# zc402/video-classification

Hardware: AMD Instinct MI355X
Metric: clips/sec SlowFast-R50 8x8, 32x224^2 bf16 training step (higher is better)
Workload: dtype bf16

## Files before the change

video-classification_amd/build.py:

```python
import os
import subprocess
from concurrent.futures import ThreadPoolExecutor

HERE = os.path.dirname(os.path.abspath(__file__))
ROOT = os.path.dirname(HERE)
CSRC = os.path.join(HERE, "csrc")
LIB = os.path.join(HERE, "libsfk.so")
SOURCES = ["conv_igemm.hip", "conv_igemm_p8.hip", "conv_halo.hip", "conv_pw.hip", "conv_wgrad.hip", "conv_wgrad_p8.hip", "conv_wgrad_band.hip", "stem_conv.hip", "bn.hip", "bn_tail.hip", "pool_head.hip",
           "optim_misc.hip", "eval_input.hip", "stem2d.hip", "roi_resize.hip", "sgd.hip", "color_jitter.hip", "u8_pool_gather.hip", "pad_resize.hip", "optim_sched.hip", "optim_groups.hip"]


def _newer(a, b):
    return (not os.path.exists(b)) or os.path.getmtime(a) > os.path.getmtime(b)


def build(force: bool = False, verbose: bool = False) -> str:
    hipcc = os.environ.get("HIPCC", "/opt/rocm/bin/hipcc")
    if not os.path.exists(hipcc):
        hipcc = "hipcc"
    objdir = os.path.join(HERE, "build")
    os.makedirs(objdir, exist_ok=True)
    deps = [os.path.join(CSRC, "sfk_common.h"), os.path.join(CSRC, "conv_igemm_epi.h"), os.path.join(CSRC, "conv_wgrad_common.h"), os.path.join(CSRC, "conv_wgrad_band_acc.inc"), os.path.join(ROOT, "include", "sfk.h"),
            os.path.join(ROOT, "include", "sfk_stem2d.h"), os.path.join(ROOT, "include", "sfk_u8stem.h"),
            os.path.join(ROOT, "include", "sfk_v2.h"), os.path.join(ROOT, "include", "sfk_aug.h"),
            os.path.join(ROOT, "include", "sfk_pool.h"), os.path.join(ROOT, "include", "sfk_resize.h"),
            os.path.join(ROOT, "include", "sfk_resident.h"), os.path.join(ROOT, "include", "sfk_roi_pool.h"),
            os.path.join(ROOT, "include", "sfk_roi_ragged.h"), os.path.join(ROOT, "include", "sfk_u8stem_pool.h"),
            os.path.join(ROOT, "include", "sfk_optim.h"), os.path.join(ROOT, "include", "sfk_groups.h"),
            os.path.join(CSRC, "optim_elem.h")]
    flags = ["--offload-arch=gfx950", "-O3", "-fPIC", "-std=c++17", "-I" + os.path.join(ROOT, "include"), "-I" + CSRC]
    flags += os.environ.get("SFK_EXTRA_FLAGS", "").split()

    def compile_one(src):
        s = os.path.join(CSRC, src)
        o = os.path.join(objdir, src.replace(".hip", ".o"))
        if force or _newer(s, o) or any(_newer(d, o) for d in deps):
            cmd = [hipcc] + flags + ["-c", s, "-o", o]
            if verbose:
                print(" ".join(cmd))
            subprocess.run(cmd, check=True)
            return o, True
        return o, False

    with ThreadPoolExecutor(max_workers=min(4, len(SOURCES))) as ex:
        res = list(ex.map(compile_one, SOURCES))
    objs = [o for o, _ in res]
    if force or any(ch for _, ch in res) or not os.path.exists(LIB):
        subprocess.run([hipcc, "--offload-arch=gfx950", "-shared", "-fPIC", "-o", LIB] + objs, check=True)
    return LIB


if __name__ == "__main__":
    print(build(force="--force" in os.sys.argv, verbose=True))
```

video-classification_amd/csrc/bn.hip:

```cpp
#include "sfk_common.h"


namespace {
inline int nt_hint(const sfk_fmap* f, int64_t mb, int bits) {
  const int64_t bytes = sfk_fmap_pixels(f) * f->c * (f->dtype == SFK_BF16 ? 2 : 4);
  return (mb >= 0 && bytes >= (mb << 20)) ? bits : 0;
}

struct FM {
  void* p;
  int ld, off;
};
inline FM fm_of(const sfk_fmap* f) { return FM{f ? f->ptr : nullptr, f ? f->ld : 0, f ? f->c_off : 0}; }

struct ChanMap {
  int cg, row, rows_b;
  bool active;
  __device__ __forceinline__ ChanMap(int cgs) {
    const int cgs_b = cgs < 256 ? cgs : 256;
    rows_b = 256 / cgs_b;
    const int tx = threadIdx.x % cgs_b, ty = threadIdx.x / cgs_b;
    cg = blockIdx.y * 256 + tx;
    row = ty;
    active = ty < rows_b && cg < cgs;
  }
};

#ifndef SFK_BN_U_ROWS
#define SFK_BN_U_ROWS 4
#endif
constexpr int SFK_BN_U = SFK_BN_U_ROWS;
inline unsigned span_blocks(int cgs, int64_t pixels) {
  const int cgs_b = cgs < 256 ? cgs : 256, rows_b = 256 / cgs_b;
  const int64_t want = (pixels + (int64_t)rows_b * SFK_BN_U - 1) / ((int64_t)rows_b * SFK_BN_U);
  return (unsigned)(want < 65535 ? (want > 0 ? want : 1) : 65535);
}
inline dim3 chan_grid(int cgs, int64_t pixels, int max_parts, int* nparts) {
  const int cgs_b = cgs < 256 ? cgs : 256;
  const int rows_b = 256 / cgs_b;
  int64_t parts = (pixels + (int64_t)rows_b * 16 - 1) / ((int64_t)rows_b * 16);
  const int cchunks = (cgs + 255) / 256;
  const int cap_all = sfk_tune().bn_parts;
  int64_t cap = cap_all / cchunks;
  if (cap < 1) cap = 1;
  if (parts > cap) parts = cap;
  if (max_parts > 0 && parts > max_parts) parts = max_parts;
  if (parts < 1) parts = 1;
  *nparts = (int)parts;
  return dim3((unsigned)parts, (unsigned)cchunks);
}

template <int VEC>
__device__ __forceinline__ void load_coef(float (&dst)[VEC], const float* src, int cg) {
#pragma unroll
  for (int i = 0; i < VEC; ++i) dst[i] = src[cg * VEC + i];
}

template <int VEC>
__device__ __forceinline__ void block_reduce_store(const ChanMap& cm, int cgs, const float (&a)[VEC],
                                                   const float (&b)[VEC], float* partials, int c) {
  __shared__ float red[256 * 2 * VEC];
  float* mine = red + threadIdx.x * 2 * VEC;
#pragma unroll
  for (int i = 0; i < VEC; ++i) {
    mine[2 * i] = cm.active ? a[i] : 0.f;
    mine[2 * i + 1] = cm.active ? b[i] : 0.f;
  }
  __syncthreads();
  const int cgs_b = cgs < 256 ? cgs : 256;
  const int W = cgs_b * 2 * VEC, rows = cm.rows_b, tid = threadIdx.x;
  float* out = partials + (int64_t)blockIdx.x * c * 2 + (int64_t)blockIdx.y * 256 * VEC * 2;
  const int ncol = (cgs - (int)blockIdx.y * 256 < cgs_b ? cgs - (int)blockIdx.y * 256 : cgs_b) * 2 * VEC;
  if (W >= 256) {
    for (int col = tid; col < W; col += 256) {
      float sacc = 0.f;
      for (int r = 0; r < rows; ++r) sacc += red[r * W + col];
      if (col < ncol) out[col] = sacc;
    }
    return;
  }
  const int G = 256 / W;
  const int g = tid / W, col = tid - g * W;
  float sacc = 0.f;
// ... 429 lines not shown
        c1[i] = coef[(cm.cg * VEC + i) * 3 + 1];
        c2[i] = coef[(cm.cg * VEC + i) * 3 + 2];
      }
    }
    const T* gp = static_cast<const T*>(dout.p) + dout.off + cm.cg * VEC;
    const uint8_t* ap = argmax + cm.cg * VEC;
    const T* yp = static_cast<const T*>(y.p) + y.off + cm.cg * VEC;
    T* op = APPLY ? static_cast<T*>(dyo.p) + dyo.off + cm.cg * VEC : nullptr;
    for (int64_t q = (int64_t)blockIdx.x * cm.rows_b + cm.row; q < quads; q += (int64_t)gridDim.x * cm.rows_b) {
      uint32_t q1, b, nt, a;
      g.dqw.divmod((uint32_t)q, q1, b);
      g.dqh.divmod(q1, nt, a);
      Vec16<T> gw[4], v[4];
      uint32_t alo[4], ahi[4];
      bool wok[4], pok[4];
#pragma unroll
      for (int wa = 0; wa < 2; ++wa)
#pragma unroll
        for (int wb = 0; wb < 2; ++wb) {
          const int ho = (int)a + wa, wo = (int)b + wb, k = 2 * wa + wb;
          wok[k] = ho < g.Ho && wo < g.Wo;
          const int hc = ho < g.Ho ? ho : g.Ho - 1, wc = wo < g.Wo ? wo : g.Wo - 1;
          const int64_t opix = ((int64_t)nt * g.Ho + hc) * g.Wo + wc;
          gw[k].load(gp + opix * dout.ld);
          const uint8_t* aq = ap + opix * c;
          if (VEC == 8) {
            const uint2 a2 = *reinterpret_cast<const uint2*>(aq);
            alo[k] = a2.x;
            ahi[k] = a2.y;
          } else {
            alo[k] = *reinterpret_cast<const uint32_t*>(aq);
            ahi[k] = 0;
          }
        }
      int64_t ipix[4];
#pragma unroll
      for (int ra = 0; ra < 2; ++ra)
#pragma unroll
        for (int rb = 0; rb < 2; ++rb) {
          const int hi = 2 * (int)a + ra, wi = 2 * (int)b + rb, k = 2 * ra + rb;
          pok[k] = hi < g.H && wi < g.W;
          const int hc = hi < g.H ? hi : g.H - 1, wc = wi < g.W ? wi : g.W - 1;
          ipix[k] = ((int64_t)nt * g.H + hc) * g.W + wc;
          v[k].load(yp + ipix[k] * y.ld);
        }
#pragma unroll
      for (int ra = 0; ra < 2; ++ra)
#pragma unroll
        for (int rb = 0; rb < 2; ++rb) {
          const int k = 2 * ra + rb;
          if (!pok[k]) continue;
          Vec16<T> da, o;
#pragma unroll
          for (int i = 0; i < VEC; ++i) {
            float acc = 0.f;
#pragma unroll
            for (int wa = 0; wa <= ra; ++wa)
#pragma unroll
              for (int wb = 0; wb <= rb; ++wb) {
                const int w4 = 2 * wa + wb;
                const uint32_t code = (uint32_t)((1 + ra - 2 * wa) * 3 + (1 + rb - 2 * wb));
                const uint32_t am = ((i < 4 ? alo[w4] : ahi[w4]) >> (8 * (i & 3))) & 0xFFu;
                if (wok[w4] && am == code) acc += gw[w4].get(i);
              }
            da.set(i, acc);
          }
#pragma unroll
          for (int i = 0; i < VEC; ++i) {
            const float yv = v[k].get(i);
            const float dz = (yv * sc[i] + sh[i] > 0.f) ? da.get(i) : 0.f;
            const float xh = (yv - mu[i]) * is[i];
            if (APPLY) {
              o.set(i, c0[i] * (dz - c1[i] - xh * c2[i]));
            } else {
              s1[i] += dz;
              s2[i] += dz * xh;
            }
          }
          if (APPLY) o.store(op + ipix[k] * dyo.ld);
        }
    }
  }
  if (!APPLY) block_reduce_store<VEC>(cm, cgs, s1, s2, partials, c);
}

bool same_shape(const sfk_fmap* a, const sfk_fmap* b) {
  return a->n == b->n && a->t == b->t && a->h == b->h && a->w == b->w && a->c == b->c && a->dtype == b->dtype;
}

}

extern "C" int sfk_bn_stats(const sfk_fmap* y, float* partials, int32_t max_parts, int32_t* nparts_out,
                            sfk_stream_t stream) {
  if (!sfk_fmap_ok(y) || !partials || !nparts_out || max_parts <= 0) return SFK_ERR_INVALID;
  if (!sfk_fmap_vec_ok(y)) return SFK_ERR_UNSUPPORTED;
  const int64_t px = sfk_fmap_pixels(y);
  int np;
  const dim3 grid = chan_grid(y->c / sfk_vec_of(y->dtype), px, max_parts, &np);
  hipStream_t s = static_cast<hipStream_t>(stream);
  if (y->dtype == SFK_BF16) hipLaunchKernelGGL(bn_stats_kernel<bf16_t>, grid, dim3(256), 0, s, fm_of(y), px, y->c, partials);
  else hipLaunchKernelGGL(bn_stats_kernel<float>, grid, dim3(256), 0, s, fm_of(y), px, y->c, partials);
  SFK_CHECK_LAUNCH();
  *nparts_out = np;
  return SFK_OK;
}

extern "C" int sfk_bn_finalize(const float* partials, int32_t nparts, int32_t c, int64_t count, const float* gamma,
                               const float* beta, float eps, float momentum, float* running_mean,
                               float* running_var, int64_t* num_batches_tracked, float* mean, float* invstd,
                               float* scale, float* shift, float* workspace, sfk_stream_t stream) {
  if (!partials || nparts <= 0 || c <= 0 || count <= 0 || !gamma || !beta || !mean || !invstd || !scale || !shift)
    return SFK_ERR_INVALID;
  if ((running_mean == nullptr) != (running_var == nullptr)) return SFK_ERR_INVALID;
  if (c & 1) return SFK_ERR_UNSUPPORTED;
  if ((((uintptr_t)partials) | ((uintptr_t)workspace)) & 15) return SFK_ERR_INVALID;
  hipStream_t s = static_cast<hipStream_t>(stream);
  partials = fold_partials(partials, nparts, c, workspace, &nparts, s);
  const FinK f{partials, nparts, c, (double)count, gamma, beta, eps, momentum, running_mean, running_var, num_batches_tracked,
               mean, invstd, scale, shift};
  hipLaunchKernelGGL(bn_finalize_kernel, dim3(c / 2), dim3(256), 0, s, f);
  SFK_CHECK_LAUNCH();
  return SFK_OK;
}

extern "C" int sfk_bn_eval_coeffs(const float* gamma, const float* beta, const float* running_mean,
                                  const float* running_var, float eps, int32_t c, float* scale, float* shift,
                                  sfk_stream_t stream) {
  if (!gamma || !beta || !running_mean || !running_var || !scale || !shift || c <= 0) return SFK_ERR_INVALID;
  hipLaunchKernelGGL(bn_eval_coeffs_kernel, dim3((c + 63) / 64), dim3(64), 0, static_cast<hipStream_t>(stream), gamma,
                     beta, running_mean, running_var, eps, c, scale, shift);
  SFK_CHECK_LAUNCH();
  return SFK_OK;
}

namespace {
template <typename T>
int launch_apply(const sfk_fmap* y, const float* scale, const float* shift, const sfk_fmap* res,
                 const float* rs, const float* rb, int relu, const sfk_fmap* out, uint8_t* bits, float* sums, int max_parts,
                 int* nparts_out, hipStream_t s) {
  const int64_t px = sfk_fmap_pixels(y);
  int np;
  dim3 grid = chan_grid(y->c / DT<T>::VEC, px, sums ? max_parts : 0, &np);
  const dim3 blk(256);
  const FM fy = fm_of(y), fr = fm_of(res), fo = fm_of(out);
  const int mode = !res ? 0 : (rs ? 2 : 1);
  const int nt = nt_hint(y, sfk_tune().nt_apply_mb, 3);
  if (sums) {
    if (mode != 0 || !relu) return SFK_ERR_UNSUPPORTED;
    if (nt) hipLaunchKernelGGL((bn_apply_kernel<T, 0, true, 3, true>), grid, blk, 0, s, fy, fr, fo, px, y->c, scale, shift, rs, rb, bits, sums);
    else hipLaunchKernelGGL((bn_apply_kernel<T, 0, true, 0, true>), grid, blk, 0, s, fy, fr, fo, px, y->c, scale, shift, rs, rb, bits, sums);
    SFK_CHECK_LAUNCH();
    *nparts_out = np;
    return SFK_OK;
  }
  grid.x = span_blocks(y->c / DT<T>::VEC, px);
#define SFK_APPLY(R, A)                                                                                                      \
  do {                                                                                                                     \
    if (nt) hipLaunchKernelGGL((bn_apply_kernel<T, R, A, 3>), grid, blk, 0, s, fy, fr, fo, px, y->c, scale, shift, rs, rb, bits); \
    else hipLaunchKernelGGL((bn_apply_kernel<T, R, A, 0>), grid, blk, 0, s, fy, fr, fo, px, y->c, scale, shift, rs, rb, bits);    \
  } while (0)
  if (relu) {
    if (mode == 0) SFK_APPLY(0, true); else if (mode == 1) SFK_APPLY(1, true); else SFK_APPLY(2, true);
  } else {
    if (mode == 0) SFK_APPLY(0, false); else if (mode == 1) SFK_APPLY(1, false); else SFK_APPLY(2, false);
  }
#undef SFK_APPLY
// ... 108 lines not shown
                                   float* workspace, sfk_stream_t stream) {
  if (!partials || nparts <= 0 || c <= 0 || count <= 0 || !gamma || !invstd || !coef) return SFK_ERR_INVALID;
  if (c & 1) return SFK_ERR_UNSUPPORTED;
  if ((((uintptr_t)partials) | ((uintptr_t)workspace)) & 15) return SFK_ERR_INVALID;
  hipStream_t s = static_cast<hipStream_t>(stream);
  partials = fold_partials(partials, nparts, c, workspace, &nparts, s);
  const BFinK f{partials, nparts, c, (double)count, gamma, invstd, dgamma, dbeta, coef};
  hipLaunchKernelGGL(bn_bwd_finalize_kernel, dim3(c / 2), dim3(256), 0, s, f);
  SFK_CHECK_LAUNCH();
  return SFK_OK;
}

extern "C" int sfk_bn_bwd_apply(const sfk_fmap* da, const sfk_fmap* y, const sfk_fmap* mask_src, const float* mean,
                                const float* invstd, const float* scale, const float* shift, int32_t relu,
                                const float* coef, const sfk_fmap* dy, sfk_stream_t stream) {
  const int st = check_bwd(da, y, mask_src, mean, invstd, scale, shift, relu);
  if (st != SFK_OK) return st;
  if (!coef || !sfk_fmap_ok(dy) || !same_shape(da, dy)) return SFK_ERR_INVALID;
  if (!sfk_fmap_vec_ok(dy)) return SFK_ERR_UNSUPPORTED;
  hipStream_t s = static_cast<hipStream_t>(stream);
  return y->dtype == SFK_BF16
             ? launch_bwd_apply<bf16_t>(da, y, mask_src, mean, invstd, scale, shift, relu, coef, dy, s)
             : launch_bwd_apply<float>(da, y, mask_src, mean, invstd, scale, shift, relu, coef, dy, s);
}

namespace {
int bn_pool_check(const sfk_fmap* d_out, const uint8_t* argmax, const sfk_fmap* y, const float* mean, const float* invstd,
                  const float* scale, const float* shift) {
  if (!sfk_fmap_ok(d_out) || !sfk_fmap_ok(y) || !argmax || !mean || !invstd || !scale || !shift) return SFK_ERR_INVALID;
  if (d_out->dtype != y->dtype || d_out->n != y->n || d_out->t != y->t || d_out->c != y->c) return SFK_ERR_INVALID;
  if (d_out->h != (y->h + 2 - 3) / 2 + 1 || d_out->w != (y->w + 2 - 3) / 2 + 1) return SFK_ERR_INVALID;
  if (!sfk_fmap_vec_ok(d_out) || !sfk_fmap_vec_ok(y)) return SFK_ERR_UNSUPPORTED;
  if (sfk_fmap_pixels(y) >= (1ll << 31)) return SFK_ERR_UNSUPPORTED;
  return SFK_OK;
}
inline PoolGeo pool_geo(const sfk_fmap* d_out, const sfk_fmap* y) {
  PoolGeo g;
  g.H = y->h; g.W = y->w; g.Ho = d_out->h; g.Wo = d_out->w;
  g.qh = (y->h + 1) / 2; g.qw = (y->w + 1) / 2;
  g.dqw.set(g.qw); g.dqh.set(g.qh);
  return g;
}
inline int64_t pool_quads(const sfk_fmap* y, const PoolGeo& g) { return (int64_t)y->n * y->t * g.qh * g.qw; }
}

extern "C" int sfk_bn_maxpool_bwd_reduce(const sfk_fmap* d_out, const uint8_t* argmax, const sfk_fmap* y, const float* mean,
                                         const float* invstd, const float* scale, const float* shift, float* partials,
                                         int32_t max_parts, int32_t* nparts_out, sfk_stream_t stream) {
  const int st = bn_pool_check(d_out, argmax, y, mean, invstd, scale, shift);
  if (st != SFK_OK) return st;
  if (!partials || !nparts_out || max_parts <= 0) return SFK_ERR_INVALID;
  const int64_t px = sfk_fmap_pixels(y);
  int np;
  const dim3 grid = chan_grid(y->c / sfk_vec_of(y->dtype), px, max_parts, &np);
  hipStream_t s = static_cast<hipStream_t>(stream);
  const PoolGeo g = pool_geo(d_out, y);
  const int64_t quads = pool_quads(y, g);
  if (y->dtype == SFK_BF16)
    hipLaunchKernelGGL((bn_pool_bwd_kernel<bf16_t, false>), grid, dim3(256), 0, s, fm_of(d_out), argmax, fm_of(y), FM{nullptr, 0, 0},
                       quads, y->c, g, mean, invstd, scale, shift, nullptr, partials);
  else
    hipLaunchKernelGGL((bn_pool_bwd_kernel<float, false>), grid, dim3(256), 0, s, fm_of(d_out), argmax, fm_of(y), FM{nullptr, 0, 0},
                       quads, y->c, g, mean, invstd, scale, shift, nullptr, partials);
  SFK_CHECK_LAUNCH();
  *nparts_out = np;
  return SFK_OK;
}

extern "C" int sfk_bn_maxpool_bwd_apply(const sfk_fmap* d_out, const uint8_t* argmax, const sfk_fmap* y, const float* mean,
                                        const float* invstd, const float* scale, const float* shift, const float* coef,
                                        const sfk_fmap* dy, sfk_stream_t stream) {
  const int st = bn_pool_check(d_out, argmax, y, mean, invstd, scale, shift);
  if (st != SFK_OK) return st;
  if (!coef || !sfk_fmap_ok(dy) || !same_shape(y, dy)) return SFK_ERR_INVALID;
  if (!sfk_fmap_vec_ok(dy)) return SFK_ERR_UNSUPPORTED;
  const int cgs = y->c / sfk_vec_of(y->dtype);
  const int cgs_b = cgs < 256 ? cgs : 256, rows_b = 256 / cgs_b;
  const PoolGeo g = pool_geo(d_out, y);
  const int64_t quads = pool_quads(y, g);
  int64_t want = (quads + rows_b - 1) / rows_b;
  if (want > 65535 * 16) want = 65535 * 16;
  const dim3 grid((unsigned)(want > 0 ? want : 1), (unsigned)((cgs + 255) / 256));
  hipStream_t s = static_cast<hipStream_t>(stream);
  if (y->dtype == SFK_BF16)
    hipLaunchKernelGGL((bn_pool_bwd_kernel<bf16_t, true>), grid, dim3(256), 0, s, fm_of(d_out), argmax, fm_of(y), fm_of(dy), quads,
                       y->c, g, mean, invstd, scale, shift, coef, nullptr);
  else
    hipLaunchKernelGGL((bn_pool_bwd_kernel<float, true>), grid, dim3(256), 0, s, fm_of(d_out), argmax, fm_of(y), fm_of(dy), quads,
                       y->c, g, mean, invstd, scale, shift, coef, nullptr);
  SFK_CHECK_LAUNCH();
  return SFK_OK;
}
```

video-classification_amd/csrc/pool_head.hip:

```cpp
#include "sfk_common.h"

namespace {

struct FM {
  void* p;
  int t, h, w, ld, off;
};
inline FM fm_of(const sfk_fmap* f) { return FM{f->ptr, f->t, f->h, f->w, f->ld, f->c_off}; }

template <typename T, int KC = 0, int SC = 0, int PC = 0, bool BN = false>
__global__ __launch_bounds__(256) void maxpool_fwd_kernel(FM x, FM y, uint8_t* argmax, int n, int c, int k_, int s_,
                                                          int p_, FastDiv dcg, FastDiv dwo, FastDiv dho,
                                                          const float* __restrict__ scale,
                                                          const float* __restrict__ shift) {
  const int k = KC ? KC : k_, s = KC ? SC : s_, p = KC ? PC : p_;
  constexpr int VEC = DT<T>::VEC;
  const int cgs = c / VEC;
  const int64_t total = (int64_t)n * y.t * y.h * y.w * cgs;
  for (int64_t idx = (int64_t)blockIdx.x * 256 + threadIdx.x; idx < total; idx += (int64_t)gridDim.x * 256) {
    uint32_t pix, cg, q1, wo, nt, ho;
    dcg.divmod((uint32_t)idx, pix, cg);
    dwo.divmod(pix, q1, wo);
    dho.divmod(q1, nt, ho);
    float best[VEC];
    int arg[VEC];
    float sc[VEC], sh[VEC];
#pragma unroll
    for (int i = 0; i < VEC; ++i) {
      best[i] = -INFINITY;
      arg[i] = 0;
      sc[i] = BN ? scale[cg * VEC + i] : 1.f;
      sh[i] = BN ? shift[cg * VEC + i] : 0.f;
    }
    bool first = true;
    if (KC) {
      Vec16<T> v[(KC ? KC : 1) * (KC ? KC : 1)];
#pragma unroll
      for (int kh = 0; kh < (KC ? KC : 1); ++kh)
#pragma unroll
        for (int kw = 0; kw < (KC ? KC : 1); ++kw) {
          int hi = (int)ho * s - p + kh, wi = (int)wo * s - p + kw;
          hi = hi < 0 ? 0 : (hi >= x.h ? x.h - 1 : hi);
          wi = wi < 0 ? 0 : (wi >= x.w ? x.w - 1 : wi);
          v[kh * (KC ? KC : 1) + kw].load(static_cast<const T*>(x.p) + (((int64_t)nt * x.h + hi) * x.w + wi) * x.ld + x.off + cg * VEC);
        }
#pragma unroll
      for (int kh = 0; kh < (KC ? KC : 1); ++kh)
#pragma unroll
        for (int kw = 0; kw < (KC ? KC : 1); ++kw) {
          const int hi = (int)ho * s - p + kh, wi = (int)wo * s - p + kw;
          const bool in = (unsigned)hi < (unsigned)x.h && (unsigned)wi < (unsigned)x.w;
          Vec16<T> act;
          if (BN) {
#pragma unroll
            for (int i = 0; i < VEC; ++i) act.set(i, fmaxf(v[kh * (KC ? KC : 1) + kw].get(i) * sc[i] + sh[i], 0.f));
          }
#pragma unroll
          for (int i = 0; i < VEC; ++i) {
            const float f = BN ? act.get(i) : v[kh * (KC ? KC : 1) + kw].get(i);
            if (in && (first || f > best[i] || f != f)) { best[i] = f; arg[i] = kh * k + kw; }
          }
          first = first && !in;
        }
    } else
    for (int kh = 0; kh < k; ++kh) {
      const int hi = (int)ho * s - p + kh;
      if ((unsigned)hi >= (unsigned)x.h) continue;
      for (int kw = 0; kw < k; ++kw) {
        const int wi = (int)wo * s - p + kw;
        if ((unsigned)wi >= (unsigned)x.w) continue;
        Vec16<T> v;
        v.load(static_cast<const T*>(x.p) + (((int64_t)nt * x.h + hi) * x.w + wi) * x.ld + x.off + cg * VEC);
        if (BN) {
#pragma unroll
          for (int i = 0; i < VEC; ++i) v.set(i, fmaxf(v.get(i) * sc[i] + sh[i], 0.f));
        }
#pragma unroll
        for (int i = 0; i < VEC; ++i) {
          const float f = v.get(i);
          if (first || f > best[i] || f != f) { best[i] = f; arg[i] = kh * k + kw; }
        }
        first = false;
      }
    }
    Vec16<T> o;
#pragma unroll
    for (int i = 0; i < VEC; ++i) o.set(i, best[i]);
    o.store(static_cast<T*>(y.p) + (int64_t)pix * y.ld + y.off + cg * VEC);
    uint32_t lo = 0, hi = 0;
#pragma unroll
    for (int i = 0; i < VEC; ++i) {
      if (i < 4) lo |= (uint32_t)arg[i] << (8 * i);
      else hi |= (uint32_t)arg[i] << (8 * (i - 4));
    }
    uint8_t* ap = argmax + (int64_t)pix * c + cg * VEC;
    if (VEC == 8) *reinterpret_cast<uint2*>(ap) = make_uint2(lo, hi);
    else *reinterpret_cast<uint32_t*>(ap) = lo;
  }
}

template <typename T, int KC = 0, int SC = 0, int PC = 0>
__global__ __launch_bounds__(256) void maxpool_bwd_kernel(FM dy, const uint8_t* argmax, FM dx, int n, int c, int k_,
                                                          int s_, int p_, FastDiv dcg, FastDiv dwi, FastDiv dhi) {
  const int k = KC ? KC : k_, s = KC ? SC : s_, p = KC ? PC : p_;
  constexpr int VEC = DT<T>::VEC;
  const int cgs = c / VEC;
  const int64_t total = (int64_t)n * dx.t * dx.h * dx.w * cgs;
  for (int64_t idx = (int64_t)blockIdx.x * 256 + threadIdx.x; idx < total; idx += (int64_t)gridDim.x * 256) {
    uint32_t pix, cg, q1, wi, nt, hi;
    dcg.divmod((uint32_t)idx, pix, cg);
    dwi.divmod(pix, q1, wi);
    dhi.divmod(q1, nt, hi);
    float acc[VEC];
#pragma unroll
    for (int i = 0; i < VEC; ++i) acc[i] = 0.f;
    if (KC == 3 && SC == 2 && PC == 1) {
      const int kh0 = ((int)hi + 1) & 1, kw0 = ((int)wi + 1) & 1;
      const int ho0 = ((int)hi + 1 - kh0) >> 1, wo0 = ((int)wi + 1 - kw0) >> 1;
      Vec16<T> g[4];
      uint32_t alo[4], ahi[4];
      bool ok[4];
      int code[4];
#pragma unroll
      for (int a = 0; a < 2; ++a)
#pragma unroll
        for (int b = 0; b < 2; ++b) {
          const int ho = ho0 - a, wo = wo0 - b, kh = kh0 + 2 * a, kw = kw0 + 2 * b;
          ok[2 * a + b] = kh < 3 && kw < 3 && ho >= 0 && wo >= 0 && ho < dy.h && wo < dy.w;
          code[2 * a + b] = kh * 3 + kw;
          const int hc = ho < 0 ? 0 : (ho >= dy.h ? dy.h - 1 : ho), wc = wo < 0 ? 0 : (wo >= dy.w ? dy.w - 1 : wo);
          const int64_t opix = ((int64_t)nt * dy.h + hc) * dy.w + wc;
          g[2 * a + b].load(static_cast<const T*>(dy.p) + opix * dy.ld + dy.off + cg * VEC);
          const uint8_t* ap = argmax + opix * c + cg * VEC;
          if (VEC == 8) {
            const uint2 a2 = *reinterpret_cast<const uint2*>(ap);
            alo[2 * a + b] = a2.x; ahi[2 * a + b] = a2.y;
          } else {
            alo[2 * a + b] = *reinterpret_cast<const uint32_t*>(ap); ahi[2 * a + b] = 0;
          }
        }
#pragma unroll
      for (int q = 0; q < 4; ++q)
#pragma unroll
        for (int i = 0; i < VEC; ++i) {
          const uint32_t am = ((i < 4 ? alo[q] : ahi[q]) >> (8 * (i & 3))) & 0xFFu;
          if (ok[q] && am == (uint32_t)code[q]) acc[i] += g[q].get(i);
        }
    } else
    for (int kh = 0; kh < k; ++kh) {
      const int num_h = (int)hi + p - kh;
      if (num_h < 0 || num_h % s) continue;
      const int ho = num_h / s;
      if (ho >= dy.h) continue;
      for (int kw = 0; kw < k; ++kw) {
        const int num_w = (int)wi + p - kw;
        if (num_w < 0 || num_w % s) continue;
        const int wo = num_w / s;
        if (wo >= dy.w) continue;
        const int64_t opix = ((int64_t)nt * dy.h + ho) * dy.w + wo;
        Vec16<T> g;
        g.load(static_cast<const T*>(dy.p) + opix * dy.ld + dy.off + cg * VEC);
        const uint8_t* ap = argmax + opix * c + cg * VEC;
        uint32_t lo, hi = 0;
        if (VEC == 8) {
          const uint2 a2 = *reinterpret_cast<const uint2*>(ap);
          lo = a2.x; hi = a2.y;
        } else {
          lo = *reinterpret_cast<const uint32_t*>(ap);
        }
#pragma unroll
        for (int i = 0; i < VEC; ++i) {
          const uint32_t a = ((i < 4 ? lo : hi) >> (8 * (i & 3))) & 0xFFu;
          if (a == (uint32_t)(kh * k + kw)) acc[i] += g.get(i);
        }
      }
    }
    Vec16<T> o;
#pragma unroll
    for (int i = 0; i < VEC; ++i) o.set(i, acc[i]);
    o.store(static_cast<T*>(dx.p) + (int64_t)pix * dx.ld + dx.off + cg * VEC);
// ... 182 lines not shown
  float s = 0.f, sb = 0.f;
  for (int ni = 0; ni < n; ++ni) {
    const float d = dl[ni * k + ki];
    s += d * feat[(int64_t)ni * f + fi];
    sb += d;
  }
  dw[idx] += s;
  if (fi == 0 && db) db[ki] += sb;
}

__global__ __launch_bounds__(256) void softmax_ce_kernel(const float* logits, const int64_t* labels, int n, int k,
                                                         float gscale, float* dlogits, float* loss_out,
                                                         float* loss_sum, int* correct) {
  __shared__ float sred[256];
  __shared__ int sidx[256];
  const int ni = blockIdx.x, tid = threadIdx.x;
  const float* lp = logits + (int64_t)ni * k;
  float mx = -INFINITY;
  int mi = 0x7fffffff;
  for (int i = tid; i < k; i += 256) {
    const float v = lp[i];
    if (v > mx) { mx = v; mi = i; }
  }
  sred[tid] = mx;
  sidx[tid] = mi;
  __syncthreads();
  for (int s = 128; s > 0; s >>= 1) {
    if (tid < s) {
      const float o = sred[tid + s];
      const int oi = sidx[tid + s];
      if (o > sred[tid] || (o == sred[tid] && oi < sidx[tid])) { sred[tid] = o; sidx[tid] = oi; }
    }
    __syncthreads();
  }
  mx = sred[0];
  const int amax = sidx[0];
  __syncthreads();
  float se = 0.f;
  for (int i = tid; i < k; i += 256) se += expf(lp[i] - mx);
  sred[tid] = se;
  __syncthreads();
  for (int s = 128; s > 0; s >>= 1) {
    if (tid < s) sred[tid] += sred[tid + s];
    __syncthreads();
  }
  se = sred[0];
  const int lab = (int)labels[ni];
  const float inv_n = 1.f / (float)n;
  if (dlogits)
    for (int i = tid; i < k; i += 256)
      dlogits[(int64_t)ni * k + i] = (expf(lp[i] - mx) / se - (i == lab ? 1.f : 0.f)) * inv_n * gscale;
  if (tid == 0) {
    const float loss = (logf(se) + mx - lp[lab]) * inv_n;
    if (loss_out) atomicAdd(loss_out, loss);
    if (loss_sum) atomicAdd(loss_sum, loss);
    if (correct && amax == lab) atomicAdd(correct, 1);
  }
}

inline unsigned grid_for(int64_t total) {
  int64_t b = (total + 255) / 256;
  const int64_t cap = sfk_tune().pool_blocks;
  if (b > cap) b = cap;
  if (b < 1) b = 1;
  return (unsigned)b;
}

}

static int maxpool_fwd_launch(const sfk_fmap* x, const float* scale, const float* shift, const sfk_fmap* y, uint8_t* argmax,
                              int32_t k, int32_t s, int32_t p, sfk_stream_t stream) {
  if (!sfk_fmap_ok(x) || !sfk_fmap_ok(y) || !argmax || k <= 0 || k > 15 || s <= 0 || p < 0) return SFK_ERR_INVALID;
  if (x->dtype != y->dtype || x->n != y->n || x->t != y->t || x->c != y->c) return SFK_ERR_INVALID;
  if (y->h != (x->h + 2 * p - k) / s + 1 || y->w != (x->w + 2 * p - k) / s + 1) return SFK_ERR_INVALID;
  if (!sfk_fmap_vec_ok(x) || !sfk_fmap_vec_ok(y)) return SFK_ERR_UNSUPPORTED;
  const int cgs = x->c / sfk_vec_of(x->dtype);
  const int64_t total = sfk_fmap_pixels(y) * cgs;
  if (total >= (1ll << 31)) return SFK_ERR_UNSUPPORTED;
  FastDiv dcg, dwo, dho;
  dcg.set(cgs); dwo.set(y->w); dho.set(y->h);
  hipStream_t st = static_cast<hipStream_t>(stream);
  const dim3 grid(grid_for(total)), blk(256);
  const bool k321 = k == 3 && s == 2 && p == 1;
#define SFK_POOL(T, K, S, P, BN) \
  hipLaunchKernelGGL((maxpool_fwd_kernel<T, K, S, P, BN>), grid, blk, 0, st, fm_of(x), fm_of(y), argmax, x->n, x->c, k, s, p, dcg, dwo, dho, scale, shift)
  if (scale) {
    if (x->dtype == SFK_BF16) { if (k321) SFK_POOL(bf16_t, 3, 2, 1, true); else SFK_POOL(bf16_t, 0, 0, 0, true); }
    else SFK_POOL(float, 0, 0, 0, true);
  } else {
    if (x->dtype == SFK_BF16) { if (k321) SFK_POOL(bf16_t, 3, 2, 1, false); else SFK_POOL(bf16_t, 0, 0, 0, false); }
    else SFK_POOL(float, 0, 0, 0, false);
  }
#undef SFK_POOL
  SFK_CHECK_LAUNCH();
  return SFK_OK;
}

extern "C" int sfk_maxpool_fwd(const sfk_fmap* x, const sfk_fmap* y, uint8_t* argmax, int32_t k, int32_t s, int32_t p,
                               sfk_stream_t stream) {
  return maxpool_fwd_launch(x, nullptr, nullptr, y, argmax, k, s, p, stream);
}

extern "C" int sfk_bn_maxpool_fwd(const sfk_fmap* y, const float* scale, const float* shift, const sfk_fmap* out,
                                  uint8_t* argmax, int32_t k, int32_t s, int32_t p, sfk_stream_t stream) {
  if (!scale || !shift) return SFK_ERR_INVALID;
  return maxpool_fwd_launch(y, scale, shift, out, argmax, k, s, p, stream);
}

extern "C" int sfk_maxpool_bwd(const sfk_fmap* dy, const uint8_t* argmax, const sfk_fmap* dx, int32_t k, int32_t s,
                               int32_t p, sfk_stream_t stream) {
  if (!sfk_fmap_ok(dx) || !sfk_fmap_ok(dy) || !argmax || k <= 0 || k > 15 || s <= 0 || p < 0) return SFK_ERR_INVALID;
  if (dx->dtype != dy->dtype || dx->n != dy->n || dx->t != dy->t || dx->c != dy->c) return SFK_ERR_INVALID;
  if (dy->h != (dx->h + 2 * p - k) / s + 1 || dy->w != (dx->w + 2 * p - k) / s + 1) return SFK_ERR_INVALID;
  if (!sfk_fmap_vec_ok(dx) || !sfk_fmap_vec_ok(dy)) return SFK_ERR_UNSUPPORTED;
  const int cgs = dx->c / sfk_vec_of(dx->dtype);
  const int64_t total = sfk_fmap_pixels(dx) * cgs;
  if (total >= (1ll << 31)) return SFK_ERR_UNSUPPORTED;
  FastDiv dcg, dwi, dhi;
  dcg.set(cgs); dwi.set(dx->w); dhi.set(dx->h);
  hipStream_t st = static_cast<hipStream_t>(stream);
  if (dx->dtype == SFK_BF16)
    if (k == 3 && s == 2 && p == 1)
      hipLaunchKernelGGL((maxpool_bwd_kernel<bf16_t, 3, 2, 1>), dim3(grid_for(total)), dim3(256), 0, st, fm_of(dy), argmax, fm_of(dx), dx->n, dx->c, k, s, p, dcg, dwi, dhi);
    else
      hipLaunchKernelGGL((maxpool_bwd_kernel<bf16_t>), dim3(grid_for(total)), dim3(256), 0, st, fm_of(dy), argmax, fm_of(dx), dx->n, dx->c, k, s, p, dcg, dwi, dhi);
  else
    hipLaunchKernelGGL((maxpool_bwd_kernel<float>), dim3(grid_for(total)), dim3(256), 0, st, fm_of(dy), argmax, fm_of(dx), dx->n, dx->c, k, s, p, dcg, dwi, dhi);
  SFK_CHECK_LAUNCH();
  return SFK_OK;
}

extern "C" int sfk_head_pool_fwd(const sfk_fmap* x, int32_t kt, int32_t kh, int32_t kw, float rate,
                                 const uint64_t* seed, float* feat, int32_t feat_ld, int32_t f_off,
                                 sfk_stream_t stream) {
  if (!sfk_fmap_ok(x) || !feat || kt <= 0 || kh <= 0 || kw <= 0 || kt > x->t || kh > x->h || kw > x->w)
    return SFK_ERR_INVALID;
  if (rate < 0.f || rate >= 1.f || (rate > 0.f && !seed) || f_off < 0 || feat_ld < f_off + x->c) return SFK_ERR_INVALID;
  hipStream_t st = static_cast<hipStream_t>(stream);
  if (kt == x->t && kh == x->h && kw == x->w && sfk_fmap_vec_ok(x)) {
    const dim3 g1((unsigned)((x->c + 255) / 256), (unsigned)x->n);
    if (x->dtype == SFK_BF16)
      hipLaunchKernelGGL(head_pool1_fwd_kernel<bf16_t>, g1, dim3(1024), 0, st, fm_of(x), x->c, rate, seed, feat, feat_ld, f_off);
    else
      hipLaunchKernelGGL(head_pool1_fwd_kernel<float>, g1, dim3(1024), 0, st, fm_of(x), x->c, rate, seed, feat, feat_ld, f_off);
    SFK_CHECK_LAUNCH();
    return SFK_OK;
  }
  const unsigned g = (unsigned)((x->n * x->c + 255) / 256);
  if (x->dtype == SFK_BF16)
    hipLaunchKernelGGL(head_pool_fwd_kernel<bf16_t>, dim3(g), dim3(256), 0, st, fm_of(x), x->n, x->c, kt, kh, kw, rate, seed, feat, feat_ld, f_off);
  else
    hipLaunchKernelGGL(head_pool_fwd_kernel<float>, dim3(g), dim3(256), 0, st, fm_of(x), x->n, x->c, kt, kh, kw, rate, seed, feat, feat_ld, f_off);
  SFK_CHECK_LAUNCH();
  return SFK_OK;
}

extern "C" int sfk_head_pool_bwd(const float* dfeat, int32_t feat_ld, int32_t f_off, int32_t kt, int32_t kh, int32_t kw,
                                 float rate, const uint64_t* seed, const sfk_fmap* dx, sfk_stream_t stream) {
  if (!sfk_fmap_ok(dx) || !dfeat || kt <= 0 || kh <= 0 || kw <= 0 || kt > dx->t || kh > dx->h || kw > dx->w)
    return SFK_ERR_INVALID;
  if (rate < 0.f || rate >= 1.f || (rate > 0.f && !seed) || f_off < 0 || feat_ld < f_off + dx->c) return SFK_ERR_INVALID;
  hipStream_t st = static_cast<hipStream_t>(stream);
  if (kt == dx->t && kh == dx->h && kw == dx->w && sfk_fmap_vec_ok(dx)) {
    const int vec = sfk_vec_of(dx->dtype), cgs = dx->c / vec;
    const int pixels = dx->t * dx->h * dx->w;
    int pxb = (pixels + 7) / 8;
// ... 56 lines not shown
```

Measured before the change: 1177.

## Add banded LDS-tiled kernels for stem BN+maxpool forward and backward

Adds two tiled kernels for the stem tail (BN+ReLU fused into a 3x3 stride-2 maxpool). Each block stages a band of activation rows (forward) or pooled gradients and argmax codes (backward) in shared memory. This lets overlapping pooling windows reuse the staged data instead of reading global memory repeatedly or using a per-pixel gather. The forward kernel packs bf16 value and tap index into one integer key to get max and argmax together, and blocks are remapped across XCDs for locality. This adds shared-memory pressure and extra edge-case logic, and the new paths are enabled by default for bf16 inputs.

Result: no change. 1176 (-0.0%).

```diff
diff --git a/video-classification_amd/build.py b/video-classification_amd/build.py
--- a/video-classification_amd/build.py
+++ b/video-classification_amd/build.py
@@ -27,7 +27,7 @@
             os.path.join(ROOT, "include", "sfk_resident.h"), os.path.join(ROOT, "include", "sfk_roi_pool.h"),
             os.path.join(ROOT, "include", "sfk_roi_ragged.h"), os.path.join(ROOT, "include", "sfk_u8stem_pool.h"),
             os.path.join(ROOT, "include", "sfk_optim.h"), os.path.join(ROOT, "include", "sfk_groups.h"),
-            os.path.join(CSRC, "optim_elem.h")]
+            os.path.join(CSRC, "optim_elem.h"), os.path.join(CSRC, "stem_tail_band.h")]
     flags = ["--offload-arch=gfx950", "-O3", "-fPIC", "-std=c++17", "-I" + os.path.join(ROOT, "include"), "-I" + CSRC]
     flags += os.environ.get("SFK_EXTRA_FLAGS", "").split()
 
diff --git a/video-classification_amd/csrc/bn.hip b/video-classification_amd/csrc/bn.hip
--- a/video-classification_amd/csrc/bn.hip
+++ b/video-classification_amd/csrc/bn.hip
@@ -1,4 +1,5 @@
 #include "sfk_common.h"
+#include "stem_tail_band.h"
 
 
 namespace {
@@ -594,6 +595,106 @@
     }
   }
   if (!APPLY) block_reduce_store<VEC>(cm, cgs, s1, s2, partials, c);
+}
+
+__global__ __launch_bounds__(256, 4) void bn_pool_band_bwd_apply_kernel(FM dout, const uint8_t* __restrict__ argmax, FM y, FM dyo,
+                                                                        int c, TailBand g, const float* mean,
+                                                                        const float* invstd, const float* scale,
+                                                                        const float* shift, const float* coef) {
+  constexpr int NWR = STB_R + 1, WPW = (NWR + 3) / 4;
+  __shared__ bf16x8 sg[NWR * STB_WSLOTS];
+  __shared__ uint2 sa[NWR * STB_WSLOTS];
+  const int lane = threadIdx.x & 63, wv = threadIdx.x >> 6;
+  const int cgl = lane & ((1 << g.lg) - 1), cg = ((int)blockIdx.y << g.lg) + cgl;
+  float mu[8], is[8], sc[8], sh[8], c0[8], c1[8], c2[8];
+  load_coef<8>(mu, mean, cg);
+  load_coef<8>(is, invstd, cg);
+  load_coef<8>(sc, scale, cg);
+  load_coef<8>(sh, shift, cg);
+#pragma unroll
+  for (int i = 0; i < 8; ++i) {
+    c0[i] = coef[(cg * 8 + i) * 3 + 0];
+    c1[i] = coef[(cg * 8 + i) * 3 + 1];
+    c2[i] = coef[(cg * 8 + i) * 3 + 2];
+  }
+  const bf16_t* gp = static_cast<const bf16_t*>(dout.p) + dout.off + cg * 8;
+  const uint8_t* ap = argmax + cg * 8;
+  const bf16_t* yp = static_cast<const bf16_t*>(y.p) + y.off + cg * 8;
+  bf16_t* op = static_cast<bf16_t*>(dyo.p) + dyo.off + cg * 8;
+  int nt, ho0, wo0, tw;
+  tail_band_tile(g, tail_band_logical(blockIdx.x, gridDim.x), nt, ho0, wo0, tw);
+  const int wcol = lane >> g.lg;
+  Vec16<bf16_t> wg[WPW];
+  uint2 wa2[WPW];
+#pragma unroll
+  for (int i = 0; i < WPW; ++i) {
+    const int ho = ho0 + wv + 4 * i, wo = wo0 + wcol;
+    const int hc = ho < g.Ho ? ho : g.Ho - 1, wc = wo < g.Wo ? wo : g.Wo - 1;
+    const int64_t opix = ((int64_t)nt * g.Ho + hc) * g.Wo + wc;
+    wg[i].load(gp + opix * dout.ld);
+    wa2[i] = *reinterpret_cast<const uint2*>(ap + opix * c);
+  }
+#pragma unroll
+  for (int i = 0; i < WPW; ++i) {
+    const int r = wv + 4 * i;
+    const bool ok = ho0 + r < g.Ho && wo0 + wcol < g.Wo;
+    if (r < NWR) {
+      sg[r * STB_WSLOTS + lane] = wg[i].v;
+      sa[r * STB_WSLOTS + lane] = ok ? wa2[i] : make_uint2(0xFFFFFFFFu, 0xFFFFFFFFu);
+    }
+  }
+  Vec16<bf16_t> v[4][2];
+  int64_t ipix[4][2];
+  bool pok[4][2];
+#pragma unroll
+  for (int i = 0; i < 4; ++i)
+#pragma unroll
+    for (int j = 0; j < 2; ++j) {
+      const int col = (lane + 64 * j) >> g.lg;
+      const int hi = 2 * ho0 + 4 * wv + i, wi = 2 * wo0 + col;
+      pok[i][j] = hi < g.H && wi < g.W && col < 2 * tw;
+      const int hc = hi < g.H ? hi : g.H - 1, wc = wi < g.W ? wi : g.W - 1;
+      ipix[i][j] = ((int64_t)nt * g.H + hc) * g.W + wc;
+      v[i][j].load(yp + ipix[i][j] * y.ld);
+    }
+  __syncthreads();
+#pragma unroll
+  for (int i = 0; i < 4; ++i)
+#pragma unroll
+    for (int j = 0; j < 2; ++j) {
+      if (!pok[i][j]) continue;
+      const int ra = i & 1;
+      const int a = 2 * wv + (i >> 1), col = (lane + 64 * j) >> g.lg, b = col >> 1, rb = col & 1;
+      float acc[8];
+#pragma unroll
+      for (int e = 0; e < 8; ++e) acc[e] = 0.f;
+#pragma unroll
+      for (int wa = 0; wa <= ra; ++wa)
+#pragma unroll
+        for (int wb = 0; wb < 2; ++wb) {
+          const uint32_t code = wb <= rb ? (uint32_t)((1 + ra - 2 * wa) * 3 + (1 + rb - 2 * wb)) : 0x100u;
+          const int ws = (a + wa) * STB_WSLOTS + ((b + wb) << g.lg) + cgl;
+          Vec16<bf16_t> gw;
+          gw.v = sg[ws];
+          const uint2 am2 = sa[ws];
+#pragma unroll
+          for (int e = 0; e < 8; ++e) {
+            const uint32_t am = ((e < 4 ? am2.x : am2.y) >> (8 * (e & 3))) & 0xFFu;
+            if (am == code) acc[e] += gw.get(e);
+          }
+        }
+      Vec16<bf16_t> da, o;
+#pragma unroll
+      for (int e = 0; e < 8; ++e) da.set(e, acc[e]);
+#pragma unroll
+      for (int e = 0; e < 8; ++e) {
+        const float yv = v[i][j].get(e);
+        const float dz = (yv * sc[e] + sh[e] > 0.f) ? da.get(e) : 0.f;
+        const float xh = (yv - mu[e]) * is[e];
+        o.set(e, c0[e] * (dz - c1[e] - xh * c2[e]));
+      }
+      o.store(op + ipix[i][j] * dyo.ld);
+    }
 }
 
 bool same_shape(const sfk_fmap* a, const sfk_fmap* b) {
@@ -868,7 +969,12 @@
   if (want > 65535 * 16) want = 65535 * 16;
   const dim3 grid((unsigned)(want > 0 ? want : 1), (unsigned)((cgs + 255) / 256));
   hipStream_t s = static_cast<hipStream_t>(stream);
-  if (y->dtype == SFK_BF16)
+  TailBand tb;
+  int slices;
+  if (SFK_STEM_TAIL_BAND && y->dtype == SFK_BF16 && tail_band_geo(y, d_out, STB_R, &tb, &slices))
+    hipLaunchKernelGGL(bn_pool_band_bwd_apply_kernel, dim3(tb.tiles, slices), dim3(256), 0, s, fm_of(d_out), argmax, fm_of(y),
+                       fm_of(dy), y->c, tb, mean, invstd, scale, shift, coef);
+  else if (y->dtype == SFK_BF16)
     hipLaunchKernelGGL((bn_pool_bwd_kernel<bf16_t, true>), grid, dim3(256), 0, s, fm_of(d_out), argmax, fm_of(y), fm_of(dy), quads,
                        y->c, g, mean, invstd, scale, shift, coef, nullptr);
   else
diff --git a/video-classification_amd/csrc/pool_head.hip b/video-classification_amd/csrc/pool_head.hip
--- a/video-classification_amd/csrc/pool_head.hip
+++ b/video-classification_amd/csrc/pool_head.hip
@@ -1,4 +1,5 @@
 #include "sfk_common.h"
+#include "stem_tail_band.h"
 
 namespace {
 
@@ -96,6 +97,86 @@
     uint8_t* ap = argmax + (int64_t)pix * c + cg * VEC;
     if (VEC == 8) *reinterpret_cast<uint2*>(ap) = make_uint2(lo, hi);
     else *reinterpret_cast<uint32_t*>(ap) = lo;
+  }
+}
+
+__global__ __launch_bounds__(256) void bn_maxpool_band_fwd_kernel(FM x, FM y, uint8_t* argmax, int c, TailBand g,
+                                                                  const float* __restrict__ scale,
+                                                                  const float* __restrict__ shift) {
+  constexpr int NR = 2 * STB_RF + 1, RPW = (NR + 3) / 4;
+  __shared__ uint4 act[NR * STB_SLOTS];
+  const int lane = threadIdx.x & 63, wv = threadIdx.x >> 6;
+  const int cgl = lane & ((1 << g.lg) - 1), cg = ((int)blockIdx.y << g.lg) + cgl;
+  int nt, ho0, wo0, tw;
+  tail_band_tile(g, tail_band_logical(blockIdx.x, gridDim.x), nt, ho0, wo0, tw);
+  const int nrp = g.Ho - ho0 < STB_RF ? g.Ho - ho0 : STB_RF;
+  const int nr = 2 * nrp + 1, ns = (2 * tw + 1) << g.lg;
+  const int hi0 = 2 * ho0 - 1, wi0 = 2 * wo0 - 1;
+  float sc[8], sh[8];
+#pragma unroll
+  for (int i = 0; i < 8; ++i) { sc[i] = scale[cg * 8 + i]; sh[i] = shift[cg * 8 + i]; }
+  const bf16_t* xp = static_cast<const bf16_t*>(x.p) + x.off + cg * 8;
+  Vec16<bf16_t> raw[RPW][2];
+#pragma unroll
+  for (int i = 0; i < RPW; ++i)
+#pragma unroll
+    for (int j = 0; j < 2; ++j) {
+      int hi = hi0 + wv + 4 * i, wi = wi0 + ((lane + 64 * j) >> g.lg);
+      hi = hi < 0 ? 0 : (hi >= x.h ? x.h - 1 : hi);
+      wi = wi < 0 ? 0 : (wi >= x.w ? x.w - 1 : wi);
+      raw[i][j].load(xp + (((int64_t)nt * x.h + hi) * x.w + wi) * x.ld);
+    }
+#pragma unroll
+  for (int i = 0; i < RPW; ++i)
+#pragma unroll
+    for (int j = 0; j < 2; ++j) {
+      const int r = wv + 4 * i, s = lane + 64 * j;
+      const bool in = (unsigned)(hi0 + r) < (unsigned)x.h && (unsigned)(wi0 + (s >> g.lg)) < (unsigned)x.w;
+      Vec16<bf16_t> a;
+#pragma unroll
+      for (int e = 0; e < 8; ++e) a.set(e, fmaxf(raw[i][j].get(e) * sc[e] + sh[e], 0.f));
+      const uint4 q = __builtin_bit_cast(uint4, a.v);
+      if (r < nr && s < ns) act[r * STB_SLOTS + s] = in ? q : make_uint4(0u, 0u, 0u, 0u);
+    }
+  __syncthreads();
+  const int wol = lane >> g.lg, wo = wo0 + wol;
+#pragma unroll
+  for (int pi = 0; pi < STB_RF / 4; ++pi) {
+    const int pr = wv + 4 * pi, ho = ho0 + pr;
+    if (pr >= nrp || wol >= tw) continue;
+    uint32_t key[8];
+#pragma unroll
+    for (int e = 0; e < 8; ++e) key[e] = 0u;
+#pragma unroll
+    for (int kh = 0; kh < 3; ++kh)
+#pragma unroll
+      for (int kw = 0; kw < 3; ++kw) {
+        const int r = 2 * pr + kh, col = 2 * wol + kw;
+        const bool in = (unsigned)(hi0 + r) < (unsigned)x.h && (unsigned)(wi0 + col) < (unsigned)x.w;
+        const uint32_t tc = in ? 15u - (uint32_t)(kh * 3 + kw) : 0u;
+        const uint4 q = act[r * STB_SLOTS + (col << g.lg) + cgl];
+        const uint32_t wd[4] = {q.x, q.y, q.z, q.w};
+#pragma unroll
+        for (int p = 0; p < 4; ++p) {
+          const uint32_t k0 = (wd[p] << 16) | tc, k1 = (wd[p] & 0xFFFF0000u) | tc;
+          key[2 * p] = k0 > key[2 * p] ? k0 : key[2 * p];
+          key[2 * p + 1] = k1 > key[2 * p + 1] ? k1 : key[2 * p + 1];
+        }
+      }
+    uint4 o;
+    o.x = (key[0] >> 16) | (key[1] & 0xFFFF0000u);
+    o.y = (key[2] >> 16) | (key[3] & 0xFFFF0000u);
+    o.z = (key[4] >> 16) | (key[5] & 0xFFFF0000u);
+    o.w = (key[6] >> 16) | (key[7] & 0xFFFF0000u);
+    const int64_t pix = ((int64_t)nt * g.Ho + ho) * g.Wo + wo;
+    *reinterpret_cast<uint4*>(static_cast<bf16_t*>(y.p) + pix * y.ld + y.off + cg * 8) = o;
+    uint32_t lo = 0, hi = 0;
+#pragma unroll
+    for (int e = 0; e < 4; ++e) {
+      lo |= (15u - (key[e] & 15u)) << (8 * e);
+      hi |= (15u - (key[e + 4] & 15u)) << (8 * e);
+    }
+    *reinterpret_cast<uint2*>(argmax + pix * c + cg * 8) = make_uint2(lo, hi);
   }
 }
 
@@ -444,6 +525,14 @@
   hipStream_t st = static_cast<hipStream_t>(stream);
   const dim3 grid(grid_for(total)), blk(256);
   const bool k321 = k == 3 && s == 2 && p == 1;
+  TailBand tb;
+  int slices;
+  if (SFK_STEM_TAIL_BAND && scale && k321 && x->dtype == SFK_BF16 && tail_band_geo(x, y, STB_RF, &tb, &slices)) {
+    hipLaunchKernelGGL(bn_maxpool_band_fwd_kernel, dim3(tb.tiles, slices), blk, 0, st, fm_of(x), fm_of(y), argmax, x->c, tb,
+                       scale, shift);
+    SFK_CHECK_LAUNCH();
+    return SFK_OK;
+  }
 #define SFK_POOL(T, K, S, P, BN) \
   hipLaunchKernelGGL((maxpool_fwd_kernel<T, K, S, P, BN>), grid, blk, 0, st, fm_of(x), fm_of(y), argmax, x->n, x->c, k, s, p, dcg, dwo, dho, scale, shift)
   if (scale) {
diff --git a/video-classification_amd/csrc/stem_tail_band.h b/video-classification_amd/csrc/stem_tail_band.h
--- /dev/null
+++ b/video-classification_amd/csrc/stem_tail_band.h
@@ -0,0 +1,54 @@
+#pragma once
+#include "sfk_common.h"
+
+#ifndef SFK_STEM_TAIL_BAND
+#define SFK_STEM_TAIL_BAND 1
+#endif
+
+constexpr int STB_R = 8;
+constexpr int STB_RF = 4;
+constexpr int STB_SLOTS = 128;
+constexpr int STB_WSLOTS = 64;
+
+struct TailBand {
+  int H, W, Ho, Wo;
+  int lg;
+  int rows;
+  int tw;
+  int tiles;
+  FastDiv dct, dnb;
+};
+
+static inline bool tail_band_geo(const sfk_fmap* y, const sfk_fmap* out, int rows, TailBand* g, int* slices) {
+  const int cgs = y->c / 8;
+  int lg = 0;
+  while (lg < 3 && (cgs & ((2 << lg) - 1)) == 0) ++lg;
+  const int twmax = ((STB_SLOTS >> lg) - 1) / 2;
+  const int nct = (out->w + twmax - 1) / twmax, nb = (out->h + rows - 1) / rows;
+  const int64_t tiles = (int64_t)y->n * y->t * nb * nct;
+  if (tiles >= (1ll << 31) || (cgs >> lg) > 65535) return false;
+  g->H = y->h; g->W = y->w; g->Ho = out->h; g->Wo = out->w;
+  g->lg = lg;
+  g->rows = rows;
+  g->tw = (out->w + nct - 1) / nct;
+  g->tiles = (int)tiles;
+  g->dct.set(nct); g->dnb.set(nb);
+  *slices = cgs >> lg;
+  return true;
+}
+
+#ifdef __HIPCC__
+__device__ __forceinline__ int tail_band_logical(int b, int nblk) {
+  const int q = nblk >> 3, r = nblk & 7, xcd = b & 7;
+  return (xcd < r ? xcd * (q + 1) : r * (q + 1) + (xcd - r) * q) + (b >> 3);
+}
+__device__ __forceinline__ void tail_band_tile(const TailBand& g, int tile, int& nt, int& ho0, int& wo0, int& tw) {
+  uint32_t q, ct, f, b;
+  g.dct.divmod((uint32_t)tile, q, ct);
+  g.dnb.divmod(q, f, b);
+  nt = (int)f;
+  ho0 = (int)b * g.rows;
+  wo0 = (int)ct * g.tw;
+  tw = g.Wo - wo0 < g.tw ? g.Wo - wo0 : g.tw;
+}
+#endif
```
